# radhofan/Fairify

Hardware: AMD Instinct MI355X
Metric: % partitions verified + partitions/sec on AC suite at 1/2/4/8 MI355X (higher is better)
Workload: dtype fp32

## Files before the change

### fairify_amd/csrc/args.h

```cpp
#pragma once
#include "common.h"

#define FA_MAX_PA 8
#define FA_MAX_RA 8
#define FA_CMAX_PA 8
#define FA_MAX_SPLIT 6

struct BoundArgs {
  const float* flat;
  const float* lo;
  const float* hi;
  const uint8_t* dead_in;
  int R;
  int symbolic;
  int G;
  int stride;
  int wstride;
  int wfloats;
  float* out_lb;
  float* out_ub;
  float* Lc; float* L0; float* Le;
  float* Uc; float* U0; float* Ue;
  float* layer_lb;
  float* layer_ub;
// ... 85 lines not shown
  const float* lo;
  const float* hi;
  const int64_t* pids;
  int P;
  int n_samples;
  uint32_t seed;
  int V;
  int npa;
  int pa_idx[FA_MAX_PA];
  const int64_t* values;
  int Pp;
  const int64_t* pairs;
  int nra;
  int ra_idx[FA_MAX_RA];
  int tau;
  int* counts;
  uint8_t* found;
  float* wit_x;
  float* wit_xp;
  float* z0;
  int* keys;
  int split;
  int S;
};

struct CertArgs {
  int Nn, n0, V, Pp, norient;
  const float *Lc, *L0, *Le, *Uc, *U0, *Ue;
  const float *Lcp, *L0p, *Lep, *Ucp, *U0p, *Uep;
  const float *olb, *oub, *olbp, *oubp;
  const float *xlo, *xhi, *xplo, *xphi;
  const int64_t* pairs;
  const int64_t* values;
  int npa;
  int pa_idx[FA_CMAX_PA];
  int nra;
  int ra_idx[FA_MAX_RA];
  float tau;
  const uint8_t* shared;
  float unit;
  float gmarg;
  float* gmin;
  float* tstar;
  uint8_t* open;
  float* score;
  int64_t* split_dim;
// ... 257 lines not shown
```

### fairify_amd/csrc/bindings.cpp

```cpp
#include <hip/hip_runtime.h>
#include <pybind11/pybind11.h>
#include <pybind11/stl.h>

#include <cmath>
#include <cstring>
#include <cstdint>
#include <stdexcept>
#include <vector>

#include "runtime_host.h"

namespace py = pybind11;

extern "C" int fa_bounds_launch(const NetDesc& net, BoundArgs args, hipStream_t stream);
extern "C" int fa_crown_phase_launch(const NetDesc& net, CrownPhaseArgs a, hipStream_t stream);
extern "C" size_t fa_crown_phase_bytes(const NetDesc& net);
extern "C" int fa_point_try_launch(const NetDesc& net, BoundArgs a, hipStream_t stream);
extern "C" int fa_forward_launch(const NetDesc& net, FwdArgs a, hipStream_t stream);
extern "C" int fa_sim_launch(const NetDesc& net, SimArgs a, hipStream_t stream);
extern "C" int fa_ascent_launch(const NetDesc& net, AscentArgs a, hipStream_t stream);
extern "C" int fa_certify_launch(CertArgs a, hipStream_t stream);
extern "C" int fa_falsify_launch(const NetDesc& net, FalsifyArgs a, hipStream_t stream);
extern "C" int fa_prune_masks_launch(const NetDesc& net, int P, const int* counts, const float* ub, int ub_stride,
                                     const uint8_t* sym_dead, uint8_t* code, int* cnt, hipStream_t stream);
extern "C" int fa_heuristic_launch(const NetDesc& net, int Pu, const int64_t* rows, const float* lb, const float* ub,
                                   int stride, const uint8_t* code, double q50, double qlo, double qhi, uint8_t* hnew,
                                   uint8_t* hmerged, int* hcnt, hipStream_t stream);
extern "C" int fa_agree_launch(const NetDesc& net, const float* flat, int Pm, const int64_t* rows, const float* lo,
                               const float* hi, const int64_t* pids, const uint8_t* dead, int S, uint32_t seed,
                               int* agree, hipStream_t stream);

extern "C" int fa_decode_launch(const DecodeDesc& d, const int64_t* ids, int P, const float* chunk_lo,
                                const float* chunk_hi, float* lo, float* hi, hipStream_t stream);
extern "C" int fa_trace_marker_launch(int tag, int* sink, hipStream_t stream);
extern "C" int fa_beta_launch(const NetDesc& nd, BetaArgs a, hipStream_t stream);
extern "C" int fa_beta_config(const NetDesc& nd, int* wpb, int* wtl, size_t* bytes);
extern "C" int fa_beta_opt16_fits(const NetDesc& nd);
extern "C" size_t fa_beta_opt16_scratch_floats(const NetDesc& nd, int R);
extern "C" int fa_beta_opt16_launch(const NetDesc& nd, BetaArgs a, float* pgsum, float* pgn, hipStream_t stream);
extern "C" int fa_beta_level16_launch(const NetDesc& nd, BetaArgs a, hipStream_t stream);
extern "C" int fa_beta_opt16_feas_launch(const NetDesc& nd, BetaArgs a, hipStream_t stream);
extern "C" int fa_beta_feas16_launch(const NetDesc& nd, BetaArgs a, hipStream_t stream);
// ... 230 lines not shown
    a.dead_in = P<const uint8_t>(dead_in);
    a.R = R;
    a.out_lb = P<float>(out_lb);
    a.out_ub = P<float>(out_ub);
    int rc = fa_point_try_launch(net.d, a, (hipStream_t)stream);
    if (rc < 0) ckl(-rc, "point_bounds");
    if (rc == 0) ckl(fa_bounds_launch(net.d, a, (hipStream_t)stream), "point_bounds(ibp)");
  });

  m.def("forward", [](const Net& net, uintptr_t flat, uintptr_t x, int B, uintptr_t dead, uintptr_t out,
                      uintptr_t stream) {
    FwdArgs a{};
    a.flat = P<const float>(flat);
    a.x = P<const float>(x);
    a.B = B;
    a.dead = P<const uint8_t>(dead);
    a.out = P<float>(out);
    ckl(fa_forward_launch(net.d, a, (hipStream_t)stream), "forward");
  });

  m.def("sim", [](const Net& net, uintptr_t flat, uintptr_t lo, uintptr_t hi, uintptr_t pids, int Pn, int n_samples,
                  uint32_t seed, int V, const std::vector<int>& pa, uintptr_t values, int Pp, uintptr_t pairs,
                  const std::vector<int>& ra, int tau, uintptr_t counts, uintptr_t found, uintptr_t wit_x,
                  uintptr_t wit_xp, uintptr_t z0, uintptr_t keys, int split, uintptr_t stream) {
    if (pa.size() > FA_MAX_PA || ra.size() > FA_MAX_RA) throw std::invalid_argument("too many PA/RA dims");
    if (split < 1 || (split > 1 && !keys)) throw std::invalid_argument("sim: split > 1 needs a keys buffer");
    SimArgs a{};
    a.flat = P<const float>(flat);
    a.lo = P<const float>(lo);
    a.hi = P<const float>(hi);
    a.pids = P<const int64_t>(pids);
    a.P = Pn;
    a.n_samples = n_samples;
    a.seed = seed;
    a.V = V;
    a.npa = (int)pa.size();
    for (size_t i = 0; i < pa.size(); ++i) a.pa_idx[i] = pa[i];
    a.values = P<const int64_t>(values);
    a.Pp = Pp;
    a.pairs = P<const int64_t>(pairs);
    a.nra = (int)ra.size();
    for (size_t i = 0; i < ra.size(); ++i) a.ra_idx[i] = ra[i];
    a.tau = tau;
    a.counts = P<int>(counts);
    a.found = P<uint8_t>(found);
    a.wit_x = P<float>(wit_x);
    a.wit_xp = P<float>(wit_xp);
    a.z0 = P<float>(z0);
    a.keys = P<int>(keys);
    a.split = split;
    ckl(fa_sim_launch(net.d, a, (hipStream_t)stream), "sim");
  });

  m.def("ascent", [](const Net& net, uintptr_t flat, uintptr_t lo, uintptr_t hi, uintptr_t x0, uintptr_t f0,
                     uintptr_t q0, int Pn, int K, int iters, int V, const std::vector<int>& pa, uintptr_t values,
                     int Pp, uintptr_t pairs, const std::vector<int>& free_dims, uintptr_t found, uintptr_t wit_x,
                     uintptr_t wit_xp, uintptr_t stream) {
    if (pa.size() > FA_MAX_PA || free_dims.size() > 64) throw std::invalid_argument("too many PA/free dims");
    AscentArgs a{};
    a.flat = P<const float>(flat);
    a.lo = P<const float>(lo);
    a.hi = P<const float>(hi);
    a.x0 = P<const float>(x0);
    a.f0 = P<const float>(f0);
    a.q0 = P<const int>(q0);
    a.P = Pn; a.K = K; a.iters = iters; a.V = V;
    a.npa = (int)pa.size();
    for (size_t i = 0; i < pa.size(); ++i) a.pa_idx[i] = pa[i];
    a.values = P<const int64_t>(values);
    a.Pp = Pp;
    a.pairs = P<const int64_t>(pairs);
    a.nfree = (int)free_dims.size();
    for (size_t i = 0; i < free_dims.size(); ++i) a.free_idx[i] = free_dims[i];
    a.found = P<uint8_t>(found);
    a.wit_x = P<float>(wit_x);
// ... 298 lines not shown
```

### fairify_amd/csrc/falsify.hip

```cpp
#include <hip/hip_runtime.h>

#include <climits>

#include "regfwd.h"

namespace {

struct FalsifyLds {
  int z0, fm, fq, zs, slo, shi, wa, wb, tlo, thi, wok, widx, sval, X, F, Q, marg, margq, misc, DK, floats;
};

__host__ __device__ inline bool fa_fals_relaxed(const FalsifyArgs& a) { return a.nra > 0 && a.tau > 0; }

__host__ __device__ inline FalsifyLds fa_falsify_lds(const FalsifyArgs& a, int n0, int wfloats) {
  FalsifyLds L;
  const int nl = a.n_local < a.n_samples ? a.n_local : a.n_samples;
  const int kw = a.walk_k < a.n_samples ? a.walk_k : a.n_samples;
  const int K = a.K < nl ? a.K : nl;
  const bool rx = fa_fals_relaxed(a);
  const int nm = 2 * a.nfree + (rx ? 2 * a.nra : 0);
  const int RV = rx ? 2 * a.V : a.V;
  int o = wfloats;
  L.z0 = o; o += a.n_samples;
  L.fm = o; o += nl;
// ... 92 lines not shown
}

}

template <int TM>
__global__ void __launch_bounds__(FA_THREADS) fa_falsify_kernel(NetDesc net, FalsifyArgs a, RegNetCfg cfg) {
  extern __shared__ __attribute__((aligned(16))) float smem[];
  const int tid = threadIdx.x, lane = tid & 63, wave = tid >> 6, col = lane & 15, grp = lane >> 4;
  const int n0 = net.dims[0];
  const int p = blockIdx.x;
  const int64_t pid = a.pids[p];
  const FalsifyLds L = fa_falsify_lds(a, n0, cfg.floats);
  float* z0 = smem + L.z0;
  float* fm = smem + L.fm;
  int* fq = (int*)(smem + L.fq);
  float* zs = smem + L.zs;
  float* s_lo = smem + L.slo;
  float* s_hi = smem + L.shi;
  int* misc = (int*)(smem + L.misc);
  const int nl = min(a.n_local, a.n_samples);
  const int V = a.V, Pp = a.Pp;
  const bool rx = fa_fals_relaxed(a);
  const int RV = rx ? 2 * V : V;
  fa_stage_wperm(net, a.flat, smem, tid, FA_THREADS);
  for (int i = tid; i < n0; i += FA_THREADS) {
    s_lo[i] = a.lo[(size_t)p * n0 + i];
    s_hi[i] = a.hi[(size_t)p * n0 + i];
  }
  if (tid == 0) {
    misc[0] = INT_MAX;
    misc[1] = 0;
  }
  __syncthreads();
  float HA[TM][4], HB[TM][4];
  for (int r0 = 0; r0 < a.n_samples; r0 += 64) {
    const int s = r0 + wave * 16 + col;
    const bool sv = s < a.n_samples;
    float Xb[TM][4];
#pragma unroll
    for (int t = 0; t < TM; ++t)
#pragma unroll
      for (int i = 0; i < 4; ++i) {
        const int k = 16 * t + 4 * grp + i;
        Xb[t][i] = (k < n0 && sv) ? fa_coord(a.seed, pid, s, k, s_lo[k], s_hi[k]) : 0.f;
      }
    for (int v2 = 0; v2 < RV; ++v2) {
      const int v = v2 < V ? v2 : v2 - V;
// ... 298 lines not shown
```

### fairify_amd/csrc/forward.hip

```cpp
#include "args.h"
#include "regfwd.h"

#include <stdlib.h>

#define FA_TR 64

__device__ void fa_tile_forward(const NetDesc& net, const float* __restrict__ flat, float* bufA, float* bufB,
                                int S, int nvalid, const uint8_t* __restrict__ dead_rows, int dead_stride,
                                int* counts, float* zout, const uint8_t* count_rows = nullptr) {
  const int tid = threadIdx.x;
  const int lane = tid & 63;
  const int wave = tid >> 6;
  for (int l = 0; l < net.n_layers; ++l) {
    const int n_in = net.dims[l];
    const int n_out = net.dims[l + 1];
    const float* __restrict__ W = flat + net.w_off[l];
    const float* __restrict__ bias = flat + net.b_off[l];
    const bool last = (l == net.n_layers - 1);
    const int noff = net.neuron_off[l];
    const int ntiles = (n_out + 15) >> 4;
    for (int t = wave; t < 4 * ntiles; t += 4) {
      const int mt = t / ntiles, nt = t % ntiles;
      const int m = mt * 16 + (lane & 15);
      const int kq = lane >> 4;
// ... 230 lines not shown
      Z = fa_mfma4(w4.w, H[t][3], Z);
    }
    if (last) {
      if (jt == 0) {
        logit = Z[0] + sb[0];
        const unsigned long long bm = __ballot(match && grp == 0 && logit != 0.f);
        if (lane == 0 && bm) atomicAdd(&cnt[noff], __popcll(bm));
      }
      continue;
    }
#pragma unroll
    for (int i = 0; i < 4; ++i) {
      const int j = 16 * jt + 4 * grp + i;
      const float h = j >= n_out ? 0.f : fmaxf(Z[i] + sb[j], 0.f);
      H2[jt][i] = h;
      const unsigned long long bm = __ballot(match && h != 0.f);
      const int c = __popcll((bm >> (16 * grp)) & 0xFFFFull);
      if (col == 0 && c) atomicAdd(&cnt[noff + j], c);
    }
  }
  return logit;
}

template <int TM>
__global__ void __launch_bounds__(FA_THREADS) fa_sim_reg_kernel(NetDesc net, SimArgs a, RegNetCfg cfg) {
  extern __shared__ __attribute__((aligned(16))) float smem[];
  const int tid = threadIdx.x, lane = tid & 63, wave = tid >> 6, col = lane & 15, grp = lane >> 4;
  const int n0 = net.dims[0];
  const int G = a.split;
  const int p = blockIdx.x / G;
  const int g = blockIdx.x - p * G;
  const int V = a.V;
  const bool rx = a.nra > 0;
  const int RV = rx ? 2 * V : V;
  const uint32_t seed_ra = a.seed ^ 0x2545F491u;
  const int64_t pid = a.pids[p];
  float* zs = smem + cfg.floats;
  float* s_lo = zs + 64 * RV;
  float* s_hi = s_lo + n0;
  int* cnt = (int*)(s_hi + n0);
  int* best = cnt + net.n_neurons;
  fa_stage_wperm(net, a.flat, smem, tid, FA_THREADS);
  for (int i = tid; i < n0; i += FA_THREADS) {
    s_lo[i] = a.lo[(size_t)p * n0 + i];
    s_hi[i] = a.hi[(size_t)p * n0 + i];
  }
  for (int i = tid; i < net.n_neurons; i += FA_THREADS) cnt[i] = 0;
  if (tid == 0) best[0] = 0x7FFFFFFF;
  __syncthreads();
  float Xb[TM][4], HA[TM][4], HB[TM][4];
  int8_t pslot[TM][4];
#pragma unroll
  for (int t = 0; t < TM; ++t)
#pragma unroll
    for (int i = 0; i < 4; ++i) {
      const int k = 16 * t + 4 * grp + i;
      int q = -1;
      for (int m = 0; m < a.npa; ++m)
        if (a.pa_idx[m] == k) q = m;
      pslot[t][i] = (int8_t)q;
    }
  for (int s0 = g * FA_TR; s0 < a.n_samples; s0 += G * FA_TR) {
    const int s = s0 + wave * 16 + col;
    const bool sv = s < a.n_samples;
#pragma unroll
    for (int t = 0; t < TM; ++t)
#pragma unroll
      for (int i = 0; i < 4; ++i) {
        const int k = 16 * t + 4 * grp + i;
        Xb[t][i] = (k < n0 && sv) ? fa_sample_coord(a.seed, pid, s, k, s_lo[k], s_hi[k]) : 0.f;
      }
    int vmatch = -1;
    if (sv) {
      float sp[FA_MAX_PA];
      for (int m = 0; m < a.npa; ++m) {
        const int d = a.pa_idx[m];
        sp[m] = fa_sample_coord(a.seed, pid, s, d, s_lo[d], s_hi[d]);
      }
      for (int v = 0; v < V && vmatch < 0; ++v) {
        bool eq = true;
        for (int m = 0; m < a.npa; ++m) eq = eq && sp[m] == (float)a.values[v * a.npa + m];
        if (eq) vmatch = v;
      }
    }
    for (int v2 = 0; v2 < RV; ++v2) {
      const int v = v2 < V ? v2 : v2 - V;
      const bool xp = v2 >= V;
      const bool match = !xp && v == vmatch;
      float vals[FA_MAX_PA];
      for (int m = 0; m < a.npa; ++m) vals[m] = (float)a.values[v * a.npa + m];
#pragma unroll
      for (int t = 0; t < TM; ++t)
#pragma unroll
        for (int i = 0; i < 4; ++i) {
          const int k = 16 * t + 4 * grp + i;
          float x = Xb[t][i];
          const int q = pslot[t][i];
          if (q >= 0) x = vals[q];
          if (xp && sv)
            for (int m = 0; m < a.nra; ++m)
              if (a.ra_idx[m] == k) x += (float)(fa_rng(seed_ra, pid, s, k) % (uint32_t)(2 * a.tau + 1)) - (float)a.tau;
          HA[t][i] = x;
        }
      float z = 0.f;
      for (int l = 0; l < net.n_layers; ++l) {
        if (l & 1) z = fa_reg_layer_count<TM>(net, cfg, smem, l, lane, HB, HA, match, cnt);
        else z = fa_reg_layer_count<TM>(net, cfg, smem, l, lane, HA, HB, match, cnt);
      }
      if (grp == 0) zs[(wave * 16 + col) * RV + v2] = z;
    }
    if (grp == 0 && sv) {
      const float* zr = zs + (wave * 16 + col) * RV;
      if (a.z0) a.z0[(size_t)p * a.n_samples + s] = zr[0];
      for (int q = 0; q < a.Pp; ++q) {
        const float zi = zr[(int)a.pairs[2 * q]], zj = zr[(rx ? V : 0) + (int)a.pairs[2 * q + 1]];
        if ((zi < 0.f && zj > 0.f) || (zi > 0.f && zj < 0.f)) {
          atomicMin(best, s * a.Pp + q);
          break;
        }
      }
    }
  }
  __syncthreads();
  const int key = best[0];
  if (G > 1) {
    for (int i = tid; i < net.n_neurons; i += FA_THREADS)
      if (cnt[i]) atomicAdd(&a.counts[(size_t)p * net.n_neurons + i], cnt[i]);
    if (tid == 0 && key != 0x7FFFFFFF) atomicMin(&a.keys[p], key);
    return;
  }
  for (int i = tid; i < net.n_neurons; i += FA_THREADS) a.counts[(size_t)p * net.n_neurons + i] = cnt[i];
  if (tid == 0) a.found[p] = key != 0x7FFFFFFF;
  if (key != 0x7FFFFFFF) fa_sim_witness(a, n0, p, pid, key, s_lo, s_hi);
}

namespace {
typedef void (*SimRegKernel)(NetDesc, SimArgs, RegNetCfg);
SimRegKernel select_sim_reg(int TM) {
  if (TM <= 1) return fa_sim_reg_kernel<1>;
  if (TM <= 2) return fa_sim_reg_kernel<2>;
  if (TM <= 4) return fa_sim_reg_kernel<4>;
  if (TM <= 7) return fa_sim_reg_kernel<7>;
  if (TM <= 10) return fa_sim_reg_kernel<10>;
  return nullptr;
}
bool sim_reg_on() {
  static const bool v = [] {
    const char* e = getenv("FAIRIFY_SIM_REG");
    return !(e && e[0] == '0');
  }();
  return v;
}
}

extern "C" int fa_sim_launch(const NetDesc& net, SimArgs a, hipStream_t stream) {
  if (a.P <= 0) return 0;
  if (a.npa > FA_MAX_PA || a.nra > FA_MAX_RA) return -3;
  if ((long long)a.n_samples * a.Pp >= 0x7FFFFFFFLL) return -3;
  a.S = net.max_width | 1;
  const int n0 = net.dims[0];
  if (sim_reg_on()) {
    const SimRegKernel k = select_sim_reg(fa_regnet_tm(net));
    RegNetCfg cfg{};
    if (k && fa_regnet_cfg(net, cfg)) {
      const size_t RV = a.nra > 0 ? 2 * (size_t)a.V : (size_t)a.V;
      size_t rb = ((size_t)cfg.floats + 64 * RV + 2 * n0) * sizeof(float) + (net.n_neurons + 4) * sizeof(int);
      rb = (rb + 15) & ~(size_t)15;
      const int tiles = (a.n_samples + FA_TR - 1) / FA_TR;
      if (rb <= 160 * 1024 && a.split >= 1 && (a.split == 1 || (a.keys && a.split <= tiles))) {
        if (!fa_lds_ok(rb)) return -4;
        hipLaunchKernelGGL(k, dim3((unsigned)a.P * (unsigned)a.split), dim3(FA_THREADS), rb, stream, net, a, cfg);
        if (a.split > 1) hipLaunchKernelGGL(fa_sim_finalize_kernel, dim3(a.P), dim3(FA_THREADS), 0, stream, net, a);
        return (int)hipGetLastError();
      }
    }
  }
  size_t floats = 2 * (size_t)FA_TR * a.S + (size_t)FA_TR * n0 + 2 * (size_t)FA_TR * a.V + FA_TR + 2 * n0;
  size_t bytes = floats * sizeof(float) + (net.n_neurons + 4) * sizeof(int) + FA_TR;
  bytes = (bytes + 15) & ~(size_t)15;
  if (bytes > 160 * 1024) return -1;
  if (!fa_lds_ok(bytes)) return -4;
  const int tiles = (a.n_samples + FA_TR - 1) / FA_TR;
  if (a.split < 1 || (a.split > 1 && (!a.keys || a.split > tiles))) return -2;
  hipLaunchKernelGGL(fa_sim_kernel, dim3((unsigned)a.P * (unsigned)a.split), dim3(FA_THREADS), bytes, stream, net, a);
  if (a.split > 1) hipLaunchKernelGGL(fa_sim_finalize_kernel, dim3(a.P), dim3(FA_THREADS), 0, stream, net, a);
// ... 112 lines not shown
    }
  }
}

extern "C" int fa_ascent_launch(const NetDesc& net, AscentArgs a, hipStream_t stream) {
  if (a.P <= 0) return 0;
  if (a.npa > FA_MAX_PA || a.nfree > 64 || a.K <= 0 || a.V <= 0 || a.Pp <= 0) return -3;
  a.S = net.max_width | 1;
  const int n0 = net.dims[0];
  const size_t nm = 2 * (size_t)a.nfree;
  const size_t floats = 2 * (size_t)FA_TR * a.S + FA_TR + (size_t)a.K * n0 + a.K + (size_t)a.K * nm * a.V +
                        (size_t)a.K * nm + 2 * (size_t)n0;
  size_t bytes = floats * sizeof(float) + ((size_t)a.K + (size_t)a.K * nm + 2) * sizeof(int);
  bytes = (bytes + 15) & ~(size_t)15;
  if (bytes > 160 * 1024) return -1;
  if (!fa_lds_ok(bytes)) return -4;
  hipLaunchKernelGGL(fa_ascent_kernel, dim3(a.P), dim3(FA_THREADS), bytes, stream, net, a);
  return (int)hipGetLastError();
}

FA_LDS_REGISTER(FA_LDS_K(fa_forward_kernel), FA_LDS_K(fa_sim_kernel), FA_LDS_K(fa_ascent_kernel),
                FA_LDS_K(fa_sim_reg_kernel<1>), FA_LDS_K(fa_sim_reg_kernel<2>), FA_LDS_K(fa_sim_reg_kernel<4>),
                FA_LDS_K(fa_sim_reg_kernel<7>), FA_LDS_K(fa_sim_reg_kernel<10>));
```

### fairify_amd/csrc/points.hip

```cpp
#include <hip/hip_runtime.h>

#include <algorithm>
#include <map>
#include <mutex>

#include "args.h"

struct PointCfg {
  int w_lds[FA_MAX_LAYERS];
  int b_lds[FA_MAX_LAYERS];
};

template <int TM>
__device__ __forceinline__ void fa_point_layer(const NetDesc& net, const BoundArgs& a, const PointCfg& cfg,
                                               const float* smem, int l, int p0, int lane,
                                               const float (&H)[TM][4], const float (&E)[TM][4],
                                               float (&H2)[TM][4], float (&E2)[TM][4]) {
  const int col = lane & 15, grp = lane >> 4;
  const int n_in = net.dims[l], n_out = net.dims[l + 1];
  const int tin = (n_in + 15) >> 4, tout = (n_out + 15) >> 4;
  const float* sw = smem + cfg.w_lds[l];
  const float* sb = smem + cfg.b_lds[l];
  const bool last = l == net.n_layers - 1;
  const float gg = net.g_fwd[l];
  const float gi = net.g_one;
  const float gnext = last ? 0.f : net.g_fwd[l + 1];
  const int noff = net.neuron_off[l];
  const int p = p0 + col;
  const bool pv = p < a.R;
#pragma unroll
  for (int jt = 0; jt < TM; ++jt) {
    if (jt >= tout) break;
    f32x4 Z = {0.f, 0.f, 0.f, 0.f}, Q = {0.f, 0.f, 0.f, 0.f};
    const float4* wq = reinterpret_cast<const float4*>(sw) + (size_t)jt * tin * 64 + lane;
#pragma unroll
    for (int t = 0; t < TM; ++t) {
      if (t >= tin) break;
      const float4 w4 = wq[t * 64];
      const float wv[4] = {w4.x, w4.y, w4.z, w4.w};
#pragma unroll
      for (int i = 0; i < 4; ++i) {
        Z = fa_mfma4(wv[i], H[t][i], Z);
        Q = fa_mfma4(fabsf(wv[i]), E[t][i], Q);
      }
    }
#pragma unroll
    for (int i = 0; i < 4; ++i) {
      const int j = 16 * jt + 4 * grp + i;
      const bool jv = j < n_out;
      const float b = jv ? sb[j] : 0.f;
      const float z = Z[i] + b;
      const float d = Q[i] * (1.f + 2.f * gg) + gg * fabsf(b) + gi * fabsf(z);
      if (last) {
        if (j == 0 && pv) {
          a.out_lb[p] = z - d;
          a.out_ub[p] = z + d;
        }
        continue;
      }
      bool forced = false;
      if (jv && pv) {
        if (a.dead_in) forced = a.dead_in[(size_t)p * net.n_hidden + noff + j] != 0;
        else if (a.dead_part)
          forced = a.dead_part[(size_t)a.node_part[a.part_mod ? p % a.part_mod : p] * net.n_hidden + noff + j] != 0;
      }
      const bool zero = !jv || forced || (z + d <= 0.f);
      const float h = zero ? 0.f : fmaxf(z, 0.f);
      const float e = zero ? 0.f : d;
      H2[jt][i] = h;
      E2[jt][i] = e + gnext * h;
    }
  }
}

template <int TM>
__global__ void __launch_bounds__(FA_THREADS) __attribute__((amdgpu_waves_per_eu(TM == 7 ? 2 : 1))) fa_point_kernel(NetDesc net, BoundArgs a, PointCfg cfg) {
  extern __shared__ __attribute__((aligned(16))) float smem[];
  const int tid = threadIdx.x;
  {
    const float4* src = reinterpret_cast<const float4*>(a.flat + net.wperm_off);
    float4* dst = reinterpret_cast<float4*>(smem);
    for (int e = tid; e < (net.wperm_floats >> 2); e += FA_THREADS) dst[e] = src[e];
  }
  __syncthreads();
  const int lane = tid & 63, col = lane & 15, grp = lane >> 4;
  const int wave = tid >> 6, nw = FA_THREADS / 64;
  const int n0 = net.dims[0];
  const int tin0 = (n0 + 15) >> 4;
  const float g0 = net.g_fwd[0];
  const int ntile = (a.R + 15) >> 4;
  for (int tile = blockIdx.x * nw + wave; tile < ntile; tile += gridDim.x * nw) {
    const int p0 = tile * 16;
    const int p = p0 + col;
    if (a.row_open && !__any(p < a.R && a.row_open[p % a.open_mod])) continue;
    float HA[TM][4], EA[TM][4], HB[TM][4], EB[TM][4];
#pragma unroll
    for (int t = 0; t < TM; ++t) {
      if (t >= tin0) break;
#pragma unroll
      for (int i = 0; i < 4; ++i) {
        const int k = 16 * t + 4 * grp + i;
        const float x = (k < n0 && p < a.R) ? a.lo[(size_t)p * n0 + k] : 0.f;
        HA[t][i] = x;
        EA[t][i] = g0 * fabsf(x);
      }
// ... 27 lines not shown
      cus = 256;
  });
  return cus;
}
}

extern "C" int fa_point_try_launch(const NetDesc& net, BoundArgs a, hipStream_t stream) {
  if (a.R <= 0) return 1;
  int TM = 1;
  for (int l = 0; l <= net.n_layers; ++l) TM = std::max(TM, (net.dims[l] + 15) / 16);
  PointKernel k = select_point(TM);
  if (!k) return 0;
  PointCfg cfg{};
  int off = 0;
  for (int l = 0; l < net.n_layers; ++l) {
    cfg.w_lds[l] = off;
    off += ((net.dims[l] + 15) / 16) * ((net.dims[l + 1] + 15) / 16) * 256;
  }
  for (int l = 0; l < net.n_layers; ++l) {
    cfg.b_lds[l] = off;
    off += net.dims[l + 1];
  }
  if (((off + 3) & ~3) != net.wperm_floats) return -1;
  const size_t bytes = (size_t)((off + 3) & ~3) * sizeof(float);
  if (bytes > 150 * 1024) return 0;
  static std::mutex mu;
  static std::map<std::pair<const void*, size_t>, int> occ;
  int per_cu = 0;
  {
    std::lock_guard<std::mutex> g(mu);
    const auto key = std::make_pair((const void*)k, bytes);
    auto it = occ.find(key);
    if (it == occ.end()) {
      if (!fa_lds_ok(bytes)) return -4;
      if (hipOccupancyMaxActiveBlocksPerMultiprocessor(&per_cu, k, FA_THREADS, bytes) != hipSuccess || per_cu <= 0)
        per_cu = 1;
      occ[key] = per_cu;
    } else {
      per_cu = it->second;
    }
  }
  const long long tiles = (a.R + 15) / 16;
  long long blocks = (tiles + 3) / 4;
  const long long cap = (long long)point_cus() * per_cu;
  if (blocks > cap) blocks = cap;
  hipLaunchKernelGGL(k, dim3((unsigned)blocks), dim3(FA_THREADS), bytes, stream, net, a, cfg);
  const hipError_t e = hipGetLastError();
  return e == hipSuccess ? 1 : -(int)e;
// ... 5 lines not shown
```

### fairify_amd/csrc/prune.hip

```cpp
#include <hip/hip_runtime.h>

#include "regfwd.h"

#define PM_CAND 1
#define PM_B 2
#define PM_S 4
#define PM_ST 8
#define PM_SCAND 16

__device__ __forceinline__ int fa_layer_end(const NetDesc& net, int l) { return net.neuron_off[l] + net.dims[l + 1]; }

__global__ void __launch_bounds__(FA_THREADS) fa_prune_masks_kernel(NetDesc net, int P, const int* counts,
                                                                   const float* ub, int ub_stride,
                                                                   const uint8_t* sym_dead, uint8_t* code,
                                                                   int* cnt) {
  const int p = blockIdx.x * FA_THREADS + threadIdx.x;
  if (p >= P) return;
  const int N = net.n_neurons, Nh = net.n_hidden;
  const int* c = counts + (size_t)p * N;
  const float* u = ub + (size_t)p * ub_stride;
  const uint8_t* sd = sym_dead ? sym_dead + (size_t)p * Nh : nullptr;
  uint8_t* out = code + (size_t)p * N;
  int nb = 0, ns = 0, nst = 0;
  for (int l = 0; l < net.n_layers; ++l) {
// ... 115 lines not shown
    __syncthreads();
  }
  if (lane == 0) {
    hcnt[2 * k + 0] = n_new;
    hcnt[2 * k + 1] = n_merged;
  }
}

template <int TM>
__global__ void __launch_bounds__(FA_THREADS) fa_agree_kernel(NetDesc net, RegNetCfg cfg, const float* flat, int Pm,
                                                              const int64_t* rows,
                                                              const float* lo, const float* hi, const int64_t* pids,
                                                              const uint8_t* dead, int S, uint32_t seed, int* agree) {
  extern __shared__ __attribute__((aligned(16))) float smem[];
  const int tid = threadIdx.x, lane = tid & 63, wave = tid >> 6, col = lane & 15, grp = lane >> 4;
  const int k = blockIdx.x;
  const int n0 = net.dims[0], Nh = net.n_hidden;
  const int64_t p = rows[k];
  const int64_t pid = pids[p];
  float* s_lo = smem + cfg.floats;
  float* s_hi = s_lo + n0;
  int* acc = (int*)(s_hi + n0);
  uint8_t* dm = (uint8_t*)(acc + 4);
  fa_stage_wperm(net, flat, smem, tid, FA_THREADS);
  for (int i = tid; i < n0; i += FA_THREADS) {
    s_lo[i] = lo[(size_t)p * n0 + i];
    s_hi[i] = hi[(size_t)p * n0 + i];
  }
  for (int i = tid; i < Nh; i += FA_THREADS) dm[i] = dead[(size_t)k * Nh + i];
  if (tid < 4) acc[tid] = 0;
  __syncthreads();
  int mine = 0, tp = 0, fp = 0;
  float HA[TM][4], HB[TM][4], X[TM][4];
  for (int s0 = wave * 16; s0 < S; s0 += 64) {
    const int s = s0 + col;
    const bool sv = s < S;
#pragma unroll
    for (int t = 0; t < TM; ++t)
#pragma unroll
      for (int i = 0; i < 4; ++i) {
        const int d = 16 * t + 4 * grp + i;
        float x = 0.f;
        if (d < n0 && sv) {
          const uint32_t h = fa_rng(seed, pid, s, d);
          x = s_lo[d] + (float)(h % ((uint32_t)(s_hi[d] - s_lo[d]) + 1u));
        }
        X[t][i] = x;
// ... 74 lines not shown
```

### fairify_amd/csrc/regfwd.h

```cpp
#pragma once
#include "args.h"

struct RegNetCfg {
  int w_lds[FA_MAX_LAYERS];
  int b_lds[FA_MAX_LAYERS];
  int floats;
};

inline bool fa_regnet_cfg(const NetDesc& net, RegNetCfg& cfg) {
  int off = 0;
  for (int l = 0; l < net.n_layers; ++l) {
    cfg.w_lds[l] = off;
    off += ((net.dims[l] + 15) / 16) * ((net.dims[l + 1] + 15) / 16) * 256;
  }
  for (int l = 0; l < net.n_layers; ++l) {
    cfg.b_lds[l] = off;
    off += net.dims[l + 1];
  }
  cfg.floats = (off + 3) & ~3;
  return cfg.floats == net.wperm_floats;
}

inline int fa_regnet_tm(const NetDesc& net) {
  int tm = 1;
  for (int l = 0; l <= net.n_layers; ++l) tm = tm > (net.dims[l] + 15) / 16 ? tm : (net.dims[l] + 15) / 16;
  return tm;
}

__device__ __forceinline__ void fa_stage_wperm(const NetDesc& net, const float* flat, float* smem, int tid,
                                               int nthreads) {
  const float4* src = reinterpret_cast<const float4*>(flat + net.wperm_off);
  float4* dst = reinterpret_cast<float4*>(smem);
  for (int e = tid; e < (net.wperm_floats >> 2); e += nthreads) dst[e] = src[e];
}

template <int TM>
__device__ __forceinline__ float fa_reg_layer(const NetDesc& net, const RegNetCfg& cfg, const float* sw_all, int l,
                                              int lane, const float (&H)[TM][4], float (&H2)[TM][4],
                                              const uint8_t* dead = nullptr) {
  const int grp = lane >> 4;
  const int n_in = net.dims[l], n_out = net.dims[l + 1];
  const int tin = (n_in + 15) >> 4, tout = (n_out + 15) >> 4;
  const float4* sw = reinterpret_cast<const float4*>(sw_all + cfg.w_lds[l]);
  const float* sb = sw_all + cfg.b_lds[l];
  const bool last = l == net.n_layers - 1;
  float logit = 0.f;
#pragma unroll
  for (int jt = 0; jt < TM; ++jt) {
    if (jt >= tout) break;
    f32x4 Z = {0.f, 0.f, 0.f, 0.f};
    const float4* wq = sw + (size_t)jt * tin * 64 + lane;
#pragma unroll
    for (int t = 0; t < TM; ++t) {
      if (t >= tin) break;
      const float4 w4 = wq[t * 64];
      Z = fa_mfma4(w4.x, H[t][0], Z);
      Z = fa_mfma4(w4.y, H[t][1], Z);
      Z = fa_mfma4(w4.z, H[t][2], Z);
      Z = fa_mfma4(w4.w, H[t][3], Z);
    }
    if (last) {
      if (jt == 0) logit = Z[0] + sb[0];
      continue;
    }
#pragma unroll
    for (int i = 0; i < 4; ++i) {
      const int j = 16 * jt + 4 * grp + i;
      const bool zero = j >= n_out || (dead && dead[net.neuron_off[l] + j]);
      H2[jt][i] = zero ? 0.f : fmaxf(Z[i] + sb[j], 0.f);
    }
  }
  return logit;
}

template <int TM>
__device__ __forceinline__ float fa_reg_forward(const NetDesc& net, const RegNetCfg& cfg, const float* sw_all,
                                                int lane, float (&HA)[TM][4], float (&HB)[TM][4],
                                                const uint8_t* dead = nullptr) {
  float z = 0.f;
  for (int l = 0; l < net.n_layers; ++l) {
    if (l & 1) z = fa_reg_layer<TM>(net, cfg, sw_all, l, lane, HB, HA, dead);
    else z = fa_reg_layer<TM>(net, cfg, sw_all, l, lane, HA, HB, dead);
  }
  return z;
}
```

### fairify_amd/ops/hip.py

```python
from __future__ import annotations

import os
import threading
from typing import Optional, Sequence

import torch

from . import ext
from . import reference as ref


def _stream(dev) -> int:
    return torch.cuda.current_stream(dev).cuda_stream


_LAZY_LOCK = threading.Lock()


def _net(be):
    n = getattr(be, "_hipnet", None)
    if n is None:
        with _LAZY_LOCK:
            n = getattr(be, "_hipnet", None)
            if n is None:
# ... 340 lines not shown
    if v is None or v.strip() == "":
        return 0
    try:
        n = int(v)
    except ValueError:
        raise ValueError(f"FAIRIFY_SIM_BLOCKS={v!r}: expected a non-negative integer") from None
    if n < 0:
        raise ValueError(f"FAIRIFY_SIM_BLOCKS={v!r}: expected a non-negative integer")
    return n


_SIM_BLOCKS = _parse_sim_blocks(os.environ.get("FAIRIFY_SIM_BLOCKS"))
_SIM_BLOCKS_ENV: Optional[str] = None


def _sim_split(P: int, n_samples: int) -> int:
    target = _SIM_BLOCKS if _SIM_BLOCKS_ENV is None else _parse_sim_blocks(os.environ.get("FAIRIFY_SIM_BLOCKS"))
    if not P or target <= P:
        return 1
    tiles = (n_samples + 63) // 64
    return max(1, min(tiles, -(-target // P)))


def simulate(be, q, lo, hi, pids, n_samples, seed, values, pairs, bisect_pairs, bisect_steps, return_z0=False):
    from ..engine.sim import SimResult, boundary_walk

    P, n0 = lo.shape
    dev = lo.device
    lo_c = _c(lo, torch.float32, (P, n0), "lo")
    hi_c = _c(hi, torch.float32, (P, n0), "hi")
    pids_c = _c(pids, torch.int64, (P,), "pids")
    V = values.shape[0]
    Pp = pairs.shape[0]
    values_c = _c(values, torch.int64, None, "values")
    pairs_c = _c(pairs, torch.int64, (Pp, 2), "pairs")
    split = _sim_split(P, n_samples)
    counts = (torch.zeros if split > 1 else torch.empty)(P, be.mlp.n_neurons, dtype=torch.int32, device=dev)
    keys = torch.full((P,), 0x7FFFFFFF, dtype=torch.int32, device=dev) if split > 1 else None
    found = torch.zeros(P, dtype=torch.uint8, device=dev)
    wx = torch.zeros(P, n0, dtype=torch.float32, device=dev)
    wxp = torch.zeros(P, n0, dtype=torch.float32, device=dev)
    z0 = torch.empty(P, n_samples, dtype=torch.float32, device=dev) if (bisect_pairs and bisect_steps) else None
    if P and n_samples:
        ext().sim(_net(be), be.flat.data_ptr(), lo_c.data_ptr(), hi_c.data_ptr(), pids_c.data_ptr(), P, n_samples,
                  int(seed) & 0xFFFFFFFF, V, list(q.pa_idx), values_c.data_ptr(), Pp, pairs_c.data_ptr(),
                  list(q.ra_idx) if q.relaxed else [], int(q.tau), counts.data_ptr(), found.data_ptr(),
                  wx.data_ptr(), wxp.data_ptr(), _ptr(z0), _ptr(keys), split, _stream(dev))
    res = SimResult(counts=counts, found=found.bool(), wit_x=wx, wit_xp=wxp)
    if z0 is not None:
        boundary_walk(be, q, lo_c, hi_c, pids_c, n_samples, seed, values_c, pairs_c, res, z0, bisect_pairs,
                      bisect_steps)
    return res


def ascent(be, q, lo, hi, x0, f0, q0, iters, values, pairs, free_dims):
    P, K, n0 = x0.shape
    dev = x0.device
    lo_c = _c(lo, torch.float32, (P, n0), "lo")
    hi_c = _c(hi, torch.float32, (P, n0), "hi")
    x0_c = _c(x0, torch.float32, (P, K, n0), "x0")
    f0_c = _c(f0, torch.float32, (P, K), "f0")
    q0_c = _c(q0, torch.int32, (P, K), "q0")
    V = values.shape[0]
    Pp = pairs.shape[0]
    values_c = _c(values, torch.int64, None, "values")
    pairs_c = _c(pairs, torch.int64, (Pp, 2), "pairs")
    found = torch.zeros(P, dtype=torch.uint8, device=dev)
    wx = torch.zeros(P, n0, dtype=torch.float32, device=dev)
    wxp = torch.zeros(P, n0, dtype=torch.float32, device=dev)
    if P == 0:
        return found.bool(), wx, wxp
    ok = ext().ascent(_net(be), be.flat.data_ptr(), lo_c.data_ptr(), hi_c.data_ptr(), x0_c.data_ptr(),
# ... 327 lines not shown
```

Baseline: 252,700.

## Specialise sim kernel per network shape with register-held activation counters

Adds compile-time shape-specialised variants of the register-MFMA simulation kernel for a fixed list of network architectures. Per-neuron activation counts are accumulated in registers and flushed once per block with shuffle reductions, instead of issuing LDS atomics on every layer. Biases are also staged into padded per-tile LDS slots so each lane loads them as one float4, and the dead-mask row pointer is hoisted in the point and forward kernels. The cost is more kernel instantiations and register pressure, plus a shape-match fallback to the generic path.

```diff
diff --git a/fairify_amd/csrc/args.h b/fairify_amd/csrc/args.h
--- a/fairify_amd/csrc/args.h
+++ b/fairify_amd/csrc/args.h
@@ -131,6 +131,7 @@
   int* keys;
   int split;
   int S;
+  int regcount;
 };
 
 struct CertArgs {
diff --git a/fairify_amd/csrc/bindings.cpp b/fairify_amd/csrc/bindings.cpp
--- a/fairify_amd/csrc/bindings.cpp
+++ b/fairify_amd/csrc/bindings.cpp
@@ -18,6 +18,7 @@
 extern "C" int fa_point_try_launch(const NetDesc& net, BoundArgs a, hipStream_t stream);
 extern "C" int fa_forward_launch(const NetDesc& net, FwdArgs a, hipStream_t stream);
 extern "C" int fa_sim_launch(const NetDesc& net, SimArgs a, hipStream_t stream);
+extern "C" int fa_sim_shaped(const NetDesc& net);
 extern "C" int fa_ascent_launch(const NetDesc& net, AscentArgs a, hipStream_t stream);
 extern "C" int fa_certify_launch(CertArgs a, hipStream_t stream);
 extern "C" int fa_falsify_launch(const NetDesc& net, FalsifyArgs a, hipStream_t stream);
@@ -294,7 +295,7 @@
   m.def("sim", [](const Net& net, uintptr_t flat, uintptr_t lo, uintptr_t hi, uintptr_t pids, int Pn, int n_samples,
                   uint32_t seed, int V, const std::vector<int>& pa, uintptr_t values, int Pp, uintptr_t pairs,
                   const std::vector<int>& ra, int tau, uintptr_t counts, uintptr_t found, uintptr_t wit_x,
-                  uintptr_t wit_xp, uintptr_t z0, uintptr_t keys, int split, uintptr_t stream) {
+                  uintptr_t wit_xp, uintptr_t z0, uintptr_t keys, int split, int regcount, uintptr_t stream) {
     if (pa.size() > FA_MAX_PA || ra.size() > FA_MAX_RA) throw std::invalid_argument("too many PA/RA dims");
     if (split < 1 || (split > 1 && !keys)) throw std::invalid_argument("sim: split > 1 needs a keys buffer");
     SimArgs a{};
@@ -321,8 +322,10 @@
     a.z0 = P<float>(z0);
     a.keys = P<int>(keys);
     a.split = split;
+    a.regcount = regcount;
     ckl(fa_sim_launch(net.d, a, (hipStream_t)stream), "sim");
   });
+  m.def("sim_shaped", [](const Net& net) { return fa_sim_shaped(net.d) != 0; });
 
   m.def("ascent", [](const Net& net, uintptr_t flat, uintptr_t lo, uintptr_t hi, uintptr_t x0, uintptr_t f0,
                      uintptr_t q0, int Pn, int K, int iters, int V, const std::vector<int>& pa, uintptr_t values,
diff --git a/fairify_amd/csrc/falsify.hip b/fairify_amd/csrc/falsify.hip
--- a/fairify_amd/csrc/falsify.hip
+++ b/fairify_amd/csrc/falsify.hip
@@ -138,7 +138,7 @@
   const int V = a.V, Pp = a.Pp;
   const bool rx = fa_fals_relaxed(a);
   const int RV = rx ? 2 * V : V;
-  fa_stage_wperm(net, a.flat, smem, tid, FA_THREADS);
+  fa_stage_wperm(net, cfg, a.flat, smem, tid, FA_THREADS);
   for (int i = tid; i < n0; i += FA_THREADS) {
     s_lo[i] = a.lo[(size_t)p * n0 + i];
     s_hi[i] = a.hi[(size_t)p * n0 + i];
diff --git a/fairify_amd/csrc/forward.hip b/fairify_amd/csrc/forward.hip
--- a/fairify_amd/csrc/forward.hip
+++ b/fairify_amd/csrc/forward.hip
@@ -276,11 +276,131 @@
   return logit;
 }
 
-template <int TM>
+template <class S>
+struct SimShape {
+  static constexpr int tiles(int l) { return (S::dim(l) + 15) / 16; }
+  static constexpr int tm() {
+    int m = 1;
+    for (int l = 0; l <= S::L; ++l) m = m > tiles(l) ? m : tiles(l);
+    return m;
+  }
+  static constexpr int w_lds(int l) {
+    int off = 0;
+    for (int k = 0; k < l; ++k) off += tiles(k) * tiles(k + 1) * 256;
+    return off;
+  }
+  static constexpr int b_lds(int l) {
+    int off = w_lds(S::L);
+    for (int k = 0; k < l; ++k) off += S::dim(k + 1);
+    return off;
+  }
+  static constexpr int bp_lds(int l) {
+    int off = (b_lds(S::L) + 3) & ~3;
+    for (int k = 0; k < l; ++k) off += 16 * tiles(k + 1);
+    return off;
+  }
+  static constexpr int neuron_off(int l) {
+    int off = 0;
+    for (int k = 0; k < l; ++k) off += S::dim(k + 1);
+    return off;
+  }
+  static constexpr int creg(int l) {
+    int off = 0;
+    for (int k = 0; k < l; ++k) off += 4 * tiles(k + 1);
+    return off;
+  }
+  static constexpr int n_creg() { return creg(S::L - 1) + 1; }
+};
+
+template <class S, int l, int TM>
+__device__ __forceinline__ float fa_reg_layers_count_shaped(const float* sw_all, int lane, float (&H)[TM][4],
+                                                            float (&H2)[TM][4], bool match,
+                                                            int (&C)[SimShape<S>::n_creg()]) {
+  using SS = SimShape<S>;
+  constexpr int n_out = S::dim(l + 1), tin = SS::tiles(l), tout = SS::tiles(l + 1);
+  const int grp = lane >> 4;
+  const float4* sw = reinterpret_cast<const float4*>(sw_all + SS::w_lds(l)) + lane;
+  const float* sb = sw_all + SS::b_lds(l);
+  if constexpr (l == S::L - 1) {
+    static_assert(n_out == 1, "one logit");
+    const float b0 = sb[0];
+    f32x4 Z = {0.f, 0.f, 0.f, 0.f};
+#pragma unroll
+    for (int t = 0; t < tin; ++t) {
+      const float4 w4 = sw[t * 64];
+      Z = fa_mfma4(w4.x, H[t][0], Z);
+      Z = fa_mfma4(w4.y, H[t][1], Z);
+      Z = fa_mfma4(w4.z, H[t][2], Z);
+      Z = fa_mfma4(w4.w, H[t][3], Z);
+    }
+    const float logit = Z[0] + b0;
+    C[SS::creg(l)] += (match && logit != 0.f) ? 1 : 0;
+    return logit;
+  } else {
+#pragma unroll
+    for (int jt = 0; jt < tout; ++jt) {
+      constexpr bool kFull = n_out % 16 == 0;
+      const bool full = kFull || jt < tout - 1;
+      const float4 b4 = *reinterpret_cast<const float4*>(sw_all + SS::bp_lds(l) + 16 * jt + 4 * grp);
+      const float b[4] = {b4.x, b4.y, b4.z, b4.w};
+      f32x4 Z = {0.f, 0.f, 0.f, 0.f};
+      const float4* wq = sw + jt * tin * 64;
+#pragma unroll
+      for (int t = 0; t < tin; ++t) {
+        const float4 w4 = wq[t * 64];
+        Z = fa_mfma4(w4.x, H[t][0], Z);
+        Z = fa_mfma4(w4.y, H[t][1], Z);
+        Z = fa_mfma4(w4.z, H[t][2], Z);
+        Z = fa_mfma4(w4.w, H[t][3], Z);
+      }
+#pragma unroll
+      for (int i = 0; i < 4; ++i) {
+        const int j = 16 * jt + 4 * grp + i;
+        float h = fmaxf(Z[i] + b[i], 0.f);
+        if (!full) h = j >= n_out ? 0.f : h;
+        H2[jt][i] = h;
+        C[SS::creg(l) + 4 * jt + i] += (match && h != 0.f) ? 1 : 0;
+      }
+    }
+    return fa_reg_layers_count_shaped<S, l + 1, TM>(sw_all, lane, H2, H, match, C);
+  }
+}
+
+template <class S, int l>
+__device__ __forceinline__ void fa_sim_flush_counts(int lane, const int (&C)[SimShape<S>::n_creg()], int* cnt) {
+  using SS = SimShape<S>;
+  const int grp = lane >> 4, col = lane & 15;
+  if constexpr (l == S::L - 1) {
+    int c = grp == 0 ? C[SS::creg(l)] : 0;
+    c += __shfl_xor(c, 1);
+    c += __shfl_xor(c, 2);
+    c += __shfl_xor(c, 4);
+    c += __shfl_xor(c, 8);
+    if (lane == 0 && c) atomicAdd(&cnt[SS::neuron_off(l)], c);
+  } else {
+    constexpr int n_out = S::dim(l + 1);
+#pragma unroll
+    for (int jt = 0; jt < SS::tiles(l + 1); ++jt)
+#pragma unroll
+      for (int i = 0; i < 4; ++i) {
+        const int j = 16 * jt + 4 * grp + i;
+        int c = C[SS::creg(l) + 4 * jt + i];
+        c += __shfl_xor(c, 1);
+        c += __shfl_xor(c, 2);
+        c += __shfl_xor(c, 4);
+        c += __shfl_xor(c, 8);
+        if (col == 0 && j < n_out && c) atomicAdd(&cnt[SS::neuron_off(l) + j], c);
+      }
+    fa_sim_flush_counts<S, l + 1>(lane, C, cnt);
+  }
+}
+
+template <int TM, class S = FaShapeAny>
 __global__ void __launch_bounds__(FA_THREADS) fa_sim_reg_kernel(NetDesc net, SimArgs a, RegNetCfg cfg) {
   extern __shared__ __attribute__((aligned(16))) float smem[];
   const int tid = threadIdx.x, lane = tid & 63, wave = tid >> 6, col = lane & 15, grp = lane >> 4;
-  const int n0 = net.dims[0];
+  constexpr bool kShaped = S::L > 0;
+  const int n0 = kShaped ? S::dim(0) : net.dims[0];
   const int G = a.split;
   const int p = blockIdx.x / G;
   const int g = blockIdx.x - p * G;
@@ -294,7 +414,7 @@
   float* s_hi = s_lo + n0;
   int* cnt = (int*)(s_hi + n0);
   int* best = cnt + net.n_neurons;
-  fa_stage_wperm(net, a.flat, smem, tid, FA_THREADS);
+  fa_stage_wperm(net, cfg, a.flat, smem, tid, FA_THREADS);
   for (int i = tid; i < n0; i += FA_THREADS) {
     s_lo[i] = a.lo[(size_t)p * n0 + i];
     s_hi[i] = a.hi[(size_t)p * n0 + i];
@@ -314,6 +434,11 @@
         if (a.pa_idx[m] == k) q = m;
       pslot[t][i] = (int8_t)q;
     }
+  int C[SimShape<S>::n_creg()];
+  if constexpr (kShaped) {
+#pragma unroll
+    for (int c = 0; c < SimShape<S>::n_creg(); ++c) C[c] = 0;
+  }
   for (int s0 = g * FA_TR; s0 < a.n_samples; s0 += G * FA_TR) {
     const int s = s0 + wave * 16 + col;
     const bool sv = s < a.n_samples;
@@ -357,9 +482,13 @@
           HA[t][i] = x;
         }
       float z = 0.f;
-      for (int l = 0; l < net.n_layers; ++l) {
-        if (l & 1) z = fa_reg_layer_count<TM>(net, cfg, smem, l, lane, HB, HA, match, cnt);
-        else z = fa_reg_layer_count<TM>(net, cfg, smem, l, lane, HA, HB, match, cnt);
+      if constexpr (kShaped) {
+        z = fa_reg_layers_count_shaped<S, 0, TM>(smem, lane, HA, HB, match, C);
+      } else {
+        for (int l = 0; l < net.n_layers; ++l) {
+          if (l & 1) z = fa_reg_layer_count<TM>(net, cfg, smem, l, lane, HB, HA, match, cnt);
+          else z = fa_reg_layer_count<TM>(net, cfg, smem, l, lane, HA, HB, match, cnt);
+        }
       }
       if (grp == 0) zs[(wave * 16 + col) * RV + v2] = z;
     }
@@ -375,6 +504,7 @@
       }
     }
   }
+  if constexpr (kShaped) fa_sim_flush_counts<S, 0>(lane, C, cnt);
   __syncthreads();
   const int key = best[0];
   if (G > 1) {
@@ -398,6 +528,38 @@
   if (TM <= 10) return fa_sim_reg_kernel<10>;
   return nullptr;
 }
+struct ShapedSim {
+  std::vector<int> dims;
+  SimRegKernel k;
+};
+template <int... D>
+ShapedSim shaped_sim() {
+  using S = FaShape<D...>;
+  return {{D...}, fa_sim_reg_kernel<SimShape<S>::tm(), S>};
+}
+#define FA_SIM_SHAPES(X)                                                                        \
+  X(13, 100, 100, 1) X(13, 100, 1) X(13, 64, 32, 16, 8, 4, 1) X(13, 64, 64, 1) X(13, 50, 1)     \
+  X(13, 16, 8, 1) X(13, 12, 12, 1) X(13, 10, 10, 10, 10, 1) X(13, 5, 5, 1) X(13, 5, 5, 5, 5, 1)   \
+  X(13, 3, 3, 3, 3, 1) X(13, 5, 5, 5, 5, 5, 5, 5, 5, 5, 1)
+SimRegKernel select_sim_shaped(const NetDesc& net) {
+#define FA_SIM_ENTRY(...) shaped_sim<__VA_ARGS__>(),
+  static const std::vector<ShapedSim> v = {FA_SIM_SHAPES(FA_SIM_ENTRY)};
+#undef FA_SIM_ENTRY
+  for (const auto& s : v) {
+    if ((int)s.dims.size() != net.n_layers + 1) continue;
+    bool same = true;
+    int noff = 0;
+    for (int l = 0; l <= net.n_layers && same; ++l) {
+      same = s.dims[l] == net.dims[l];
+      if (l < net.n_layers) {
+        same = same && net.neuron_off[l] == noff;
+        noff += s.dims[l + 1];
+      }
+    }
+    if (same) return s.k;
+  }
+  return nullptr;
+}
 bool sim_reg_on() {
   static const bool v = [] {
     const char* e = getenv("FAIRIFY_SIM_REG");
@@ -406,6 +568,8 @@
   return v;
 }
 }
+
+extern "C" int fa_sim_shaped(const NetDesc& net) { return select_sim_shaped(net) != nullptr; }
 
 extern "C" int fa_sim_launch(const NetDesc& net, SimArgs a, hipStream_t stream) {
   if (a.P <= 0) return 0;
@@ -414,7 +578,8 @@
   a.S = net.max_width | 1;
   const int n0 = net.dims[0];
   if (sim_reg_on()) {
-    const SimRegKernel k = select_sim_reg(fa_regnet_tm(net));
+    SimRegKernel k = a.regcount ? select_sim_shaped(net) : nullptr;
+    if (!k) k = select_sim_reg(fa_regnet_tm(net));
     RegNetCfg cfg{};
     if (k && fa_regnet_cfg(net, cfg)) {
       const size_t RV = a.nra > 0 ? 2 * (size_t)a.V : (size_t)a.V;
@@ -573,3 +738,6 @@
 FA_LDS_REGISTER(FA_LDS_K(fa_forward_kernel), FA_LDS_K(fa_sim_kernel), FA_LDS_K(fa_ascent_kernel),
                 FA_LDS_K(fa_sim_reg_kernel<1>), FA_LDS_K(fa_sim_reg_kernel<2>), FA_LDS_K(fa_sim_reg_kernel<4>),
                 FA_LDS_K(fa_sim_reg_kernel<7>), FA_LDS_K(fa_sim_reg_kernel<10>));
+#define FA_SIM_LDS(...) FA_LDS_K((fa_sim_reg_kernel<SimShape<FaShape<__VA_ARGS__>>::tm(), FaShape<__VA_ARGS__>>)),
+FA_LDS_REGISTER(FA_SIM_SHAPES(FA_SIM_LDS));
+#undef FA_SIM_LDS
diff --git a/fairify_amd/csrc/points.hip b/fairify_amd/csrc/points.hip
--- a/fairify_amd/csrc/points.hip
+++ b/fairify_amd/csrc/points.hip
@@ -9,6 +9,7 @@
 struct PointCfg {
   int w_lds[FA_MAX_LAYERS];
   int b_lds[FA_MAX_LAYERS];
+  int bp_lds[FA_MAX_LAYERS];
 };
 
 template <int TM>
@@ -20,7 +21,7 @@
   const int n_in = net.dims[l], n_out = net.dims[l + 1];
   const int tin = (n_in + 15) >> 4, tout = (n_out + 15) >> 4;
   const float* sw = smem + cfg.w_lds[l];
-  const float* sb = smem + cfg.b_lds[l];
+  const float* sbp = smem + cfg.bp_lds[l];
   const bool last = l == net.n_layers - 1;
   const float gg = net.g_fwd[l];
   const float gi = net.g_one;
@@ -28,9 +29,25 @@
   const int noff = net.neuron_off[l];
   const int p = p0 + col;
   const bool pv = p < a.R;
+  const bool masked = !last && (a.dead_in || a.dead_part);
+  const uint8_t* drow = nullptr;
+  if (masked && pv) {
+    if (a.dead_in) drow = a.dead_in + (size_t)p * net.n_hidden + noff;
+    else drow = a.dead_part + (size_t)a.node_part[a.part_mod ? p % a.part_mod : p] * net.n_hidden + noff;
+  }
 #pragma unroll
   for (int jt = 0; jt < TM; ++jt) {
     if (jt >= tout) break;
+    const float4 b4 = *reinterpret_cast<const float4*>(sbp + 16 * jt + 4 * grp);
+    const float bl[4] = {b4.x, b4.y, b4.z, b4.w};
+    bool forced[4] = {false, false, false, false};
+    if (masked) {
+#pragma unroll
+      for (int i = 0; i < 4; ++i) {
+        const int j = 16 * jt + 4 * grp + i;
+        forced[i] = drow && j < n_out && drow[j] != 0;
+      }
+    }
     f32x4 Z = {0.f, 0.f, 0.f, 0.f}, Q = {0.f, 0.f, 0.f, 0.f};
     const float4* wq = reinterpret_cast<const float4*>(sw) + (size_t)jt * tin * 64 + lane;
 #pragma unroll
@@ -48,9 +65,9 @@
     for (int i = 0; i < 4; ++i) {
       const int j = 16 * jt + 4 * grp + i;
       const bool jv = j < n_out;
-      const float b = jv ? sb[j] : 0.f;
+      const float b = bl[i];
       const float z = Z[i] + b;
-      const float d = Q[i] * (1.f + 2.f * gg) + gg * fabsf(b) + gi * fabsf(z);
+      const float d = fmaf(gi, fabsf(z), fmaf(Q[i], 1.f + 2.f * gg, gg * fabsf(b)));
       if (last) {
         if (j == 0 && pv) {
           a.out_lb[p] = z - d;
@@ -58,17 +75,11 @@
         }
         continue;
       }
-      bool forced = false;
-      if (jv && pv) {
-        if (a.dead_in) forced = a.dead_in[(size_t)p * net.n_hidden + noff + j] != 0;
-        else if (a.dead_part)
-          forced = a.dead_part[(size_t)a.node_part[a.part_mod ? p % a.part_mod : p] * net.n_hidden + noff + j] != 0;
-      }
-      const bool zero = !jv || forced || (z + d <= 0.f);
+      const bool zero = !jv || forced[i] || (z + d <= 0.f);
       const float h = zero ? 0.f : fmaxf(z, 0.f);
       const float e = zero ? 0.f : d;
       H2[jt][i] = h;
-      E2[jt][i] = e + gnext * h;
+      E2[jt][i] = fmaf(gnext, h, e);
     }
   }
 }
@@ -81,6 +92,11 @@
     const float4* src = reinterpret_cast<const float4*>(a.flat + net.wperm_off);
     float4* dst = reinterpret_cast<float4*>(smem);
     for (int e = tid; e < (net.wperm_floats >> 2); e += FA_THREADS) dst[e] = src[e];
+    for (int l = 0; l < net.n_layers; ++l) {
+      const int n_out = net.dims[l + 1];
+      const float* b = a.flat + net.wperm_off + cfg.b_lds[l];
+      for (int j = tid; j < ((n_out + 15) & ~15); j += FA_THREADS) smem[cfg.bp_lds[l] + j] = j < n_out ? b[j] : 0.f;
+    }
   }
   __syncthreads();
   const int lane = tid & 63, col = lane & 15, grp = lane >> 4;
@@ -154,8 +170,13 @@
     off += net.dims[l + 1];
   }
   if (((off + 3) & ~3) != net.wperm_floats) return -1;
-  const size_t bytes = (size_t)((off + 3) & ~3) * sizeof(float);
-  if (bytes > 150 * 1024) return 0;
+  if ((size_t)net.wperm_floats * sizeof(float) > 150 * 1024) return 0;
+  off = net.wperm_floats;
+  for (int l = 0; l < net.n_layers; ++l) {
+    cfg.bp_lds[l] = off;
+    off += ((net.dims[l + 1] + 15) / 16) * 16;
+  }
+  const size_t bytes = (size_t)off * sizeof(float);
   static std::mutex mu;
   static std::map<std::pair<const void*, size_t>, int> occ;
   int per_cu = 0;
diff --git a/fairify_amd/csrc/prune.hip b/fairify_amd/csrc/prune.hip
--- a/fairify_amd/csrc/prune.hip
+++ b/fairify_amd/csrc/prune.hip
@@ -161,7 +161,7 @@
   float* s_hi = s_lo + n0;
   int* acc = (int*)(s_hi + n0);
   uint8_t* dm = (uint8_t*)(acc + 4);
-  fa_stage_wperm(net, flat, smem, tid, FA_THREADS);
+  fa_stage_wperm(net, cfg, flat, smem, tid, FA_THREADS);
   for (int i = tid; i < n0; i += FA_THREADS) {
     s_lo[i] = lo[(size_t)p * n0 + i];
     s_hi[i] = hi[(size_t)p * n0 + i];
diff --git a/fairify_amd/csrc/regfwd.h b/fairify_amd/csrc/regfwd.h
--- a/fairify_amd/csrc/regfwd.h
+++ b/fairify_amd/csrc/regfwd.h
@@ -4,6 +4,7 @@
 struct RegNetCfg {
   int w_lds[FA_MAX_LAYERS];
   int b_lds[FA_MAX_LAYERS];
+  int bp_lds[FA_MAX_LAYERS];
   int floats;
 };
 
@@ -17,8 +18,14 @@
     cfg.b_lds[l] = off;
     off += net.dims[l + 1];
   }
-  cfg.floats = (off + 3) & ~3;
-  return cfg.floats == net.wperm_floats;
+  const int block = (off + 3) & ~3;
+  off = block;
+  for (int l = 0; l < net.n_layers; ++l) {
+    cfg.bp_lds[l] = off;
+    off += ((net.dims[l + 1] + 15) / 16) * 16;
+  }
+  cfg.floats = off;
+  return block == net.wperm_floats;
 }
 
 inline int fa_regnet_tm(const NetDesc& net) {
@@ -27,11 +34,16 @@
   return tm;
 }
 
-__device__ __forceinline__ void fa_stage_wperm(const NetDesc& net, const float* flat, float* smem, int tid,
-                                               int nthreads) {
+__device__ __forceinline__ void fa_stage_wperm(const NetDesc& net, const RegNetCfg& cfg, const float* flat,
+                                               float* smem, int tid, int nthreads) {
   const float4* src = reinterpret_cast<const float4*>(flat + net.wperm_off);
   float4* dst = reinterpret_cast<float4*>(smem);
   for (int e = tid; e < (net.wperm_floats >> 2); e += nthreads) dst[e] = src[e];
+  for (int l = 0; l < net.n_layers; ++l) {
+    const int n_out = net.dims[l + 1];
+    const float* b = flat + net.wperm_off + cfg.b_lds[l];
+    for (int j = tid; j < ((n_out + 15) & ~15); j += nthreads) smem[cfg.bp_lds[l] + j] = j < n_out ? b[j] : 0.f;
+  }
 }
 
 template <int TM>
@@ -43,11 +55,15 @@
   const int tin = (n_in + 15) >> 4, tout = (n_out + 15) >> 4;
   const float4* sw = reinterpret_cast<const float4*>(sw_all + cfg.w_lds[l]);
   const float* sb = sw_all + cfg.b_lds[l];
+  const float* sbp = sw_all + cfg.bp_lds[l];
   const bool last = l == net.n_layers - 1;
+  const uint8_t* dl = dead ? dead + net.neuron_off[l] : nullptr;
   float logit = 0.f;
 #pragma unroll
   for (int jt = 0; jt < TM; ++jt) {
     if (jt >= tout) break;
+    const float4 b4 = *reinterpret_cast<const float4*>(sbp + 16 * jt + 4 * grp);
+    const float b[4] = {b4.x, b4.y, b4.z, b4.w};
     f32x4 Z = {0.f, 0.f, 0.f, 0.f};
     const float4* wq = sw + (size_t)jt * tin * 64 + lane;
 #pragma unroll
@@ -63,11 +79,19 @@
       if (jt == 0) logit = Z[0] + sb[0];
       continue;
     }
+    if (dl) {
 #pragma unroll
-    for (int i = 0; i < 4; ++i) {
-      const int j = 16 * jt + 4 * grp + i;
-      const bool zero = j >= n_out || (dead && dead[net.neuron_off[l] + j]);
-      H2[jt][i] = zero ? 0.f : fmaxf(Z[i] + sb[j], 0.f);
+      for (int i = 0; i < 4; ++i) {
+        const int j = 16 * jt + 4 * grp + i;
+        const bool zero = j >= n_out || dl[j];
+        H2[jt][i] = zero ? 0.f : fmaxf(Z[i] + b[i], 0.f);
+      }
+    } else {
+#pragma unroll
+      for (int i = 0; i < 4; ++i) {
+        const int j = 16 * jt + 4 * grp + i;
+        H2[jt][i] = j >= n_out ? 0.f : fmaxf(Z[i] + b[i], 0.f);
+      }
     }
   }
   return logit;
diff --git a/fairify_amd/ops/hip.py b/fairify_amd/ops/hip.py
--- a/fairify_amd/ops/hip.py
+++ b/fairify_amd/ops/hip.py
@@ -386,6 +386,16 @@
     return max(1, min(tiles, -(-target // P)))
 
 
+_SIM_REGCOUNT = os.environ.get("FAIRIFY_SIM_REGCOUNT", "1").strip() != "0"
+_SIM_REGCOUNT_ENV: Optional[str] = None
+
+
+def _sim_regcount() -> bool:
+    if _SIM_REGCOUNT_ENV is None:
+        return _SIM_REGCOUNT
+    return os.environ.get("FAIRIFY_SIM_REGCOUNT", "1").strip() != "0"
+
+
 def simulate(be, q, lo, hi, pids, n_samples, seed, values, pairs, bisect_pairs, bisect_steps, return_z0=False):
     from ..engine.sim import SimResult, boundary_walk
 
@@ -404,14 +414,17 @@
     found = torch.zeros(P, dtype=torch.uint8, device=dev)
     wx = torch.zeros(P, n0, dtype=torch.float32, device=dev)
     wxp = torch.zeros(P, n0, dtype=torch.float32, device=dev)
-    z0 = torch.empty(P, n_samples, dtype=torch.float32, device=dev) if (bisect_pairs and bisect_steps) else None
+    walk = bool(bisect_pairs and bisect_steps)
+    z0 = torch.empty(P, n_samples, dtype=torch.float32, device=dev) if (walk or return_z0) else None
     if P and n_samples:
         ext().sim(_net(be), be.flat.data_ptr(), lo_c.data_ptr(), hi_c.data_ptr(), pids_c.data_ptr(), P, n_samples,
                   int(seed) & 0xFFFFFFFF, V, list(q.pa_idx), values_c.data_ptr(), Pp, pairs_c.data_ptr(),
                   list(q.ra_idx) if q.relaxed else [], int(q.tau), counts.data_ptr(), found.data_ptr(),
-                  wx.data_ptr(), wxp.data_ptr(), _ptr(z0), _ptr(keys), split, _stream(dev))
+                  wx.data_ptr(), wxp.data_ptr(), _ptr(z0), _ptr(keys), split, int(_sim_regcount()), _stream(dev))
     res = SimResult(counts=counts, found=found.bool(), wit_x=wx, wit_xp=wxp)
-    if z0 is not None:
+    if return_z0:
+        res.z0 = z0
+    if walk:
         boundary_walk(be, q, lo_c, hi_c, pids_c, n_samples, seed, values_c, pairs_c, res, z0, bisect_pairs,
                       bisect_steps)
     return res
```

Result: faster. 271,700, median of 6 (+7.5%).
